# anneouyang/OuterSPACE

Hardware: AMD Instinct MI355X
Metric: spgemm_output_nnz_per_s (higher is better)
Workload: dtype f64

## Files before the change

outerspace_amd/csrc/osp_kernels.h:

```cpp
#pragma once
#include <type_traits>
#include "osp_prims.h"

namespace osp {

template <class T> struct TileCap;
#ifndef OSP_TILE_CAP_F32
#define OSP_TILE_CAP_F32 1792
#endif
template <> struct TileCap<float> { static constexpr int value = OSP_TILE_CAP_F32; };
#ifndef OSP_TILE_CAP_F64
#define OSP_TILE_CAP_F64 1536
#endif
template <> struct TileCap<double> { static constexpr int value = OSP_TILE_CAP_F64; };
constexpr int kMergeThreads = 256;
constexpr int kTileMaxRows = kMergeThreads - 1;
constexpr int kMulThreads = 256;
#ifndef OSP_MUL_PER_WAVE
#define OSP_MUL_PER_WAVE 2048
#endif
constexpr int kMulPerWave = OSP_MUL_PER_WAVE;
constexpr int kMulPerBlock = kMulPerWave * (kMulThreads / kWave);
#ifndef OSP_MUL_BATCH_MAX
#define OSP_MUL_BATCH_MAX 4096
// ... 1046 lines not shown
#ifdef OSP_MERGE_PROF
__device__ unsigned long long osp_merge_prof[16];
#define OSP_PROF_DECL __shared__ unsigned long long prof_acc[12]; if (tid < 12) prof_acc[tid] = 0; __syncthreads(); unsigned long long prof_t = clock64();
#define OSP_PROF_MARK(k) do { if (tid == 0) { const unsigned long long now_ = clock64(); prof_acc[k] += now_ - prof_t; prof_t = now_; } } while (0)
#define OSP_PROF_FLUSH do { if (tid == 0) for (int k_ = 0; k_ < 12; k_++) atomicAdd(&osp_merge_prof[k_], prof_acc[k_]); } while (0)
#else
#define OSP_PROF_DECL
#define OSP_PROF_MARK(k)
#define OSP_PROF_FLUSH
#endif

constexpr int kMergeMaxWgs = 5;
#ifndef OSP_TILE_ROUNDS
#define OSP_TILE_ROUNDS 3
#endif
constexpr int kTileRoundClasses = OSP_TILE_ROUNDS > 1 ? OSP_TILE_ROUNDS : 1;
static_assert(kTileRoundClasses <= 3, "OSP_TILE_ROUNDS: at most three bodies");
constexpr int tile_class_rounds(int lpt, int c, int K) { return (lpt * c + K - 1) / K; }
template <class T, int NT, int CAP, int MAXWG = kMergeMaxWgs, int ABL = 0>
constexpr int merge_wgs_per_cu() {
    const int wgs = (160 * 1024) / (int)(sizeof(MergeSmem<T, NT, CAP>) + ((ABL & 64) ? CAP * sizeof(T) : 0) + 64);
    return wgs > MAXWG ? MAXWG : wgs;
}
template <class T, int NT, int CAP, int MAXWG = kMergeMaxWgs, int ABL = 0>
constexpr int merge_waves_per_simd() {
    const int w = (merge_wgs_per_cu<T, NT, CAP, MAXWG, ABL>() * NT + 255) / 256;
    return w > 8 ? 8 : (w < 1 ? 1 : w);
}
template <class T, int NT, int ABL = 0, int CAP = TileCap<T>::value, int MAXWG = kMergeMaxWgs, bool RA = (OSP_RANK_ATOMIC != 0), bool GA = false>
__global__ __launch_bounds__(NT, (merge_waves_per_simd<T, NT, CAP, MAXWG, ABL>())) void merge_tiles_kernel(
    const TileDesc *__restrict__ desc, uint32_t ntiles, const MergeLevels<T> lvl, int colbits, uint64_t *tile_status,
    uint32_t *ticket, const uint64_t *__restrict__ out_base_p, uint32_t *__restrict__ c_col, T *__restrict__ c_val,
    uint64_t *__restrict__ out_end_p, const ChunkTable<T> ct = ChunkTable<T>{}, uint32_t nshards = 1, uint32_t *abort_word = nullptr,
    const GatherArgs<T> ga = GatherArgs<T>{}) {
    __shared__ MergeSmem<T, NT, CAP> sm;
    __shared__ TileDesc s_dnext;
    __shared__ uint32_t s_tnext;
    constexpr bool ROWWISE = (ABL & 64) != 0;
    __shared__ T rwval[ROWWISE ? CAP : 1];
    constexpr int kTileCap = CAP;
    constexpr int NW = NT / kWave;
    constexpr int LPT = (kTileCap + NT - 1) / NT;
    constexpr int ITERS = (kTileCap / NW + kWave - 1) / kWave;
    constexpr int DPT = (kDigits + NT - 1) / NT;
    static_assert(kTileMaxRows + 1 <= NT, "row offsets are fetched one per thread");
    unsigned tid = threadIdx.x, lane = lane_id(), w = tid >> 6;
    uint32_t shard = 0;
    if constexpr (GA) { if (tid < (uint32_t)kTileCap / 32u) sm.gbits[tid] = 0; }
    if (tid == 0) {
        if (nshards > 1) shard = atomicAdd(&ticket[nshards * kTicketStride], 1u) % nshards;
        const uint32_t t0 = (ABL & 4) ? blockIdx.x : take_ticket(ticket, nshards, shard, ntiles);
        s_tnext = t0;
        if (t0 < ntiles) s_dnext = desc[t0];
    }
    __syncthreads();
#ifndef OSP_TEST_NO_LATE_GUARD
    if (s_tnext >= ntiles) return;
#endif
    const uint64_t out_base = (ABL & 32) ? 0ull : *out_base_p;
    const uint32_t colmask = colbits < 32 ? ((1u << colbits) - 1u) : 0xffffffffu;
    uint32_t t = s_tnext;
    TileDesc d = s_dnext;
    OSP_CRUMB(5, ntiles, d.lvl, d.nr);
    uint64_t ro = 0;
    PartWords<T> lrec[LPT];
    static_assert(!GA || kTileCap % (NW * kWave) == 0, "gathered tiles: a wave's span is a whole number of wave-loads");
    static_assert(ITERS <= LPT, "sort passes: a wave's share of a full tile in LPT wave-loads");
// ... 51 lines not shown
        int64_t *__restrict__ c_rowptr = lvl.c_rowptr[d.lvl];
        const bool long_row = n > (uint32_t)kTileCap;
        uint32_t tn_reg = ntiles;
        if (long_row) {
            if (w == 0) {
                const uint64_t total = lvl.heavy_nnz[d.lvl][ra];
                const uint64_t excl = (ABL & 2) ? (uint64_t)t * kTileCap : lookback_prefix(tile_status, t, total, abort_word);
                if (lane == 0) {
                    tn_reg = (ABL & 4) ? t + gridDim.x : take_ticket(ticket, nshards, shard, ntiles);
                    c_rowptr[ra] = (int64_t)(out_base + excl);
                    if (t + 1 == ntiles) *out_end_p = out_base + excl + total;
                    s_tnext = tn_reg;
                    if (tn_reg < ntiles) s_dnext = desc[tn_reg];
                }
            }
            __syncthreads();
            t = s_tnext;
            d = s_dnext;
            request(d, t < ntiles);
            __syncthreads();
            continue;
        }
        auto tile_body = [&](auto rounds_tag) __attribute__((always_inline)) {
        constexpr int Q = decltype(rounds_tag)::value;
        static_assert(Q >= 1 && Q <= LPT, "rounds of a tile body");
        constexpr int SQ = K > 1 ? Q : ITERS;
        ix0 = GA ? w * (uint32_t)(kWave * Q) + lane : tid;
        int rowbits = 0;
        while ((1u << rowbits) < nr) rowbits++;
        const bool relkey = d.kbits != 0;
        const uint32_t cbase = d.cbase;
        const int keybits = relkey ? (int)d.kbits : colbits + rowbits;
        const int nbits = (n && !(ABL & 1)) ? keybits : 0;
        constexpr uint32_t HS = MergeSmem<T, NT, CAP>::kHashWords;
        typedef MergeSmem<T, NT, CAP> Smem;
        static_assert(!OSP_HASH_IN_CNT || offsetof(Smem, cnt) + sizeof(sm.cnt) == offsetof(Smem, pos0) + 4u * HS,
                      "hash table: from pos0 through the digit counters without a gap");
        uint32_t *htab = sm.htab();
        constexpr bool INPLACE = (ABL & 32) != 0;
        const bool early = nbits > 0 && keybits < 32 && !(ABL & 2) && !(ABL & 8) && !INPLACE;
        const bool gath = GA && d.rcnt != 0;
        uint32_t kq[LPT];
        T vq[LPT];
        uint32_t rq[(LPT + 1) / 2];
        constexpr bool kRunInPad = GA && Smem::kWide;
        constexpr bool kKeepPos = GA && Smem::kWide;
        uint32_t bpos[LPT];
        constexpr uint32_t GW = GA ? (uint32_t)kTileCap : 0u;
        constexpr uint32_t HSG = HS - GW;
        uint32_t *gsrc = htab, *htab_g = htab + GW;
        if constexpr (GA) {
            if (gath) {
                static_assert(HS > 2 * GW, "gathered tiles: the run table leaves a hash table of more than two words per entry... of half the entries");
                const uint32_t R = d.rcnt, tile0 = (uint32_t)(s + base);
                const RunDesc<T> *__restrict__ gruns = d.lvl ? ga.runs : ga.runs0;
                for (uint32_t x = tid; x < R; x += NT) {
                    uint32_t dst = lrec[0].w[0], src = lrec[0].w[1];
                    if (x == tid + NT) { dst = lrec[1].w[0]; src = lrec[1].w[1]; }
                    else if (x != tid) { const RunDesc<T> rd = gruns[d.rbeg + x]; dst = rd.dst; src = rd.src; }
                    const uint32_t st = dst - tile0;
                    gsrc[x] = src - st;
                    atomicOr(&sm.gbits[st >> 5], 1u << (st & 31u));
                }
                if (early) {
                    typedef uint32_t u32x4 __attribute__((ext_vector_type(4)));
                    static_assert((offsetof(Smem, pos0) + 4u * GW) % 16 == 0, "gathered tiles: the hash table starts 16-byte aligned");
// ... 33 lines not shown
                {
                    const uint32_t nwords = w * (2u * Q);
                    static_assert((NW - 1) * 2 * LPT <= kWave, "gathered tiles: the bits before a wave's span, one word per lane");
                    cnt0 = wave_reduce_sum<uint32_t>(lane < nwords ? (uint32_t)__popc(sm.gbits[lane]) : 0u);
                    cnt0 = (uint32_t)__builtin_amdgcn_readfirstlane((int)cnt0);
                }
#pragma unroll
                for (int q = 0; q < (LPT + 1) / 2; q++) rq[q] = 0;
#pragma unroll
                for (int q = 0; q < Q; q++) {
                    const uint32_t i = ix0 + q * ixs;
                    const uint32_t wi = w * (2u * Q) + 2u * (uint32_t)q;
                    const uint32_t mlo = sm.gbits[wi], mhi = sm.gbits[wi + 1];
                    const uint32_t below = __builtin_amdgcn_mbcnt_hi(mhi, __builtin_amdgcn_mbcnt_lo(mlo, 0u));
                    const uint32_t own = ((lane < 32 ? mlo >> lane : mhi >> (lane - 32)) & 1u);
                    const uint32_t r = cnt0 + below + own - 1u;
                    cnt0 += (uint32_t)__popc(mlo) + (uint32_t)__popc(mhi);
                    bpos[q] = i < n ? gsrc[r] + i : 0u;
                    rq[q >> 1] |= (i < n ? r : 0u) << (16 * (q & 1));
                }
                uint32_t bc[LPT];
#pragma unroll
                for (int q = 0; q < Q; q++) bc[q] = ga.b_colidx[bpos[q]];
#pragma unroll
                for (int q = 0; q < Q; q++) {
                    const uint32_t i = ix0 + q * ixs;
                    if (relkey) {
                        kq[q] = bc[q] - cbase;
                    } else {
                        uint32_t lo = 0, hi = nr;
                        while (hi - lo > 1) { const uint32_t mid = (lo + hi) >> 1; if (sm.rowo[mid] <= i) lo = mid; else hi = mid; }
                        kq[q] = (colbits < 32 ? (lo << colbits) : 0u) | bc[q];
                    }
                    if (i < n) sm.key0[i] = kq[q];
                }
                OSP_PROF_MARK(11);
                if (early) {
                    uint32_t hq[LPT], oq[LPT];
#pragma unroll
                    for (int q = 0; q < Q; q++) {
                        hq[q] = (uint32_t)(((uint64_t)(kq[q] * 2654435761u) * HSG) >> 32);
                        oq[q] = kq[q];
                        if (ix0 + q * ixs < n) oq[q] = atomicCAS(&htab_g[hq[q]], 0xffffffffu, kq[q]);
                    }
#pragma unroll
                    for (int q = 0; q < Q; q++) {
                        if (ix0 + q * ixs < n) {
                            uint32_t old = oq[q], h = hq[q];
                            while (old != 0xffffffffu && old != kq[q]) {
                                h = (h + 1 == HSG) ? 0u : h + 1;
                                old = atomicCAS(&htab_g[h], 0xffffffffu, kq[q]);
                            }
                            fresh += old == 0xffffffffu;
                        }
                    }
                }
            }
        }
        if (gath) {
        } else if (rw_tile) {
            if constexpr (ROWWISE) {
                constexpr uint32_t kRwGroup = 16, kRwSteps = 4, kRwUnroll = 4;
                const uint32_t c0 = ct.rowfirst[ra], c1 = ct.rowfirst[ra + nr];
                for (uint32_t cb = c0 + w * kRwGroup; cb < c1; cb += NW * kRwGroup) {
                    const uint32_t c = cb + lane;
                    const bool cv = lane < kRwGroup && c < c1;
                    const uint64_t o0 = cv ? ct.off[c] : 0ull, o1 = cv ? ct.off[c + 1] : 0ull;
// ... 5 lines not shown
                    {
                        uint32_t lo = 0, hi = nr;
                        while (hi - lo > 1) { const uint32_t mid = (lo + hi) >> 1; if (sm.rowo[mid] <= st) lo = mid; else hi = mid; }
                        lrow = colbits < 32 ? (lo << colbits) : 0u;
                    }
                    const uint32_t nvalid = min(kRwGroup, c1 - cb);
                    const uint32_t gbeg = wave_bcast(st, 0u), gend = wave_bcast(en, nvalid - 1);
                    for (uint32_t ib0 = gbeg; ib0 < gend; ib0 += kRwUnroll * kWave) {
                        uint32_t bcol[kRwUnroll], crow[kRwUnroll];
                        T bval[kRwUnroll], cav[kRwUnroll];
#pragma unroll
                        for (uint32_t u = 0; u < kRwUnroll; u++) {
                            const uint32_t i = ib0 + u * kWave + lane;
                            uint32_t lo = 0, hi = kRwGroup;
#pragma unroll
                            for (uint32_t step = 0; step < kRwSteps; step++) {
                                const uint32_t mid = (lo + hi) >> 1;
                                const uint32_t sv = (uint32_t)__shfl((int)st, (int)mid);
                                if (sv <= i) lo = mid; else hi = mid;
                            }
                            const uint32_t cst = (uint32_t)__shfl((int)st, (int)lo);
                            const uint32_t cbs = (uint32_t)__shfl((int)bsv, (int)lo);
                            crow[u] = (uint32_t)__shfl((int)lrow, (int)lo);
                            cav[u] = __shfl(av, (int)lo);
                            const uint32_t b = i < gend ? cbs + (i - cst) : 0u;
                            bcol[u] = ct.b_colidx[b];
                            bval[u] = ct.b_vals[b];
                        }
#pragma unroll
                        for (uint32_t u = 0; u < kRwUnroll; u++) {
                            const uint32_t i = ib0 + u * kWave + lane;
                            if (i < gend) {
                                const uint32_t key = crow[u] | bcol[u];
                                sm.key0[i] = key;
                                rwval[i] = cav[u] * bval[u];
                                if (early) {
                                    uint32_t h = (uint32_t)(((uint64_t)(key * 2654435761u) * HS) >> 32);
                                    uint32_t old = atomicCAS(&htab[h], 0xffffffffu, key);
                                    while (old != 0xffffffffu && old != key) {
                                        h = (h + 1 == HS) ? 0u : h + 1;
                                        old = atomicCAS(&htab[h], 0xffffffffu, key);
                                    }
                                    fresh += old == 0xffffffffu;
                                }
                            }
                        }
                    }
                }
            }
        } else {
#pragma unroll
            for (int q = 0; q < Q; q++) {
                const uint32_t i = ix0 + q * ixs;
                kq[q] = 0;
                if (i < n) {
                    if (relkey) {
                        kq[q] = lrec[q].col() - cbase;
                    } else {
                        uint32_t lo = 0, hi = nr;
                        while (hi - lo > 1) { const uint32_t mid = (lo + hi) >> 1; if (sm.rowo[mid] <= i) lo = mid; else hi = mid; }
                        kq[q] = (colbits < 32 ? (lo << colbits) : 0u) | lrec[q].col();
                    }
                    sm.key0[i] = kq[q];
                }
            }
            if (early) {
                uint32_t hq[LPT], oq[LPT];
#pragma unroll
                for (int q = 0; q < Q; q++) {
                    hq[q] = (uint32_t)(((uint64_t)(kq[q] * 2654435761u) * HS) >> 32);
                    oq[q] = kq[q];
                    if (ix0 + q * ixs < n) oq[q] = atomicCAS(&htab[hq[q]], 0xffffffffu, kq[q]);
                }
#pragma unroll
                for (int q = 0; q < Q; q++) {
                    if (ix0 + q * ixs < n) {
                        uint32_t old = oq[q], h = hq[q];
                        while (old != 0xffffffffu && old != kq[q]) {
                            h = (h + 1 == HS) ? 0u : h + 1;
                            old = atomicCAS(&htab[h], 0xffffffffu, kq[q]);
                        }
                        fresh += old == 0xffffffffu;
                    }
                }
            }
        }
        if (early) {
            const uint32_t wsum = wave_incl_scan(fresh);
            if (lane == kWave - 1 && wsum) atomicAdd(&sm.hcount, wsum);
        }
        const uint32_t per = K > 1 ? (uint32_t)(kWave * Q) : (n + NW - 1) / NW;
        const uint32_t wbeg = min(w * per, n), wend = min(wbeg + per, n);
        int cur = 0;
        __syncthreads();
        if constexpr (GA) {
            if (gath) {
                if (tid < (uint32_t)kTileCap / 32u) sm.gbits[tid] = 0;
                if constexpr (kRunInPad) {
#pragma unroll
                    for (int q = 0; q < Q; q++) {
                        const uint32_t i = ix0 + q * ixs;
                        if (i < n) sm.pad[i] = (uint16_t)(rq[q >> 1] >> (16 * (q & 1)));
                    }
                }
            }
        }
        OSP_PROF_MARK(1);
        if (early && tid == 0) lookback_publish(tile_status, t, sm.hcount);
        OSP_PROF_MARK(2);
        const int npass = (nbits + kDigitBits - 1) / kDigitBits;
        const int pbits = npass ? (nbits + npass - 1) / npass : 0;
        const uint32_t dmask = (1u << pbits) - 1u;
        const int ndig = 1 << pbits;
        for (int pass = 0, shift = 0; pass < npass; pass++, shift += pbits) {
            uint32_t *ksrc = sm.key(cur), *kdst = sm.key(cur ^ 1);
            uint16_t *psrc = sm.pos(cur), *pdst = sm.pos(cur ^ 1);
            if constexpr (ABL & 128) {
                for (int dd = lane; dd < ndig; dd += kWave) sm.cnt[w][dd] = 0;
            } else {
                uint64_t *c64 = reinterpret_cast<uint64_t *>(sm.cnt[w]);
                for (int dd = lane; dd < (ndig + 3) / 4; dd += kWave) c64[dd] = 0ull;
            }
            uint32_t kreg[SQ], rreg[SQ];
            auto rank_span = [&](auto bits_tag) {
                constexpr int BITS = decltype(bits_tag)::value;
#pragma unroll
                for (int it = 0; it < SQ; it++) {
                    const uint32_t i = wbeg + it * kWave + lane;
                    const bool valid = i < wend;
                    kreg[it] = valid ? ksrc[i] : 0u;
                    const unsigned dg = (kreg[it] >> shift) & dmask;
                    unsigned rk, cntd;
                    wave_match_digit<BITS>(dg, valid, rk, cntd);
                    rreg[it] = 0;
                    if (valid) {
                        const uint32_t c = sm.cnt[w][dg];
                        rreg[it] = c + rk;
                        if (rk == 0) sm.cnt[w][dg] = (uint16_t)(c + cntd);
                    }
                }
            };
            if constexpr (RA) {
            {
                uint32_t(*cnt32)[kDigits / 2] = reinterpret_cast<uint32_t(*)[kDigits / 2]>(sm.cnt);
#pragma unroll
                for (int it = 0; it < SQ; it++) {
                    const uint32_t i = wbeg + it * kWave + lane;
// ... 36 lines not shown
                const bool on = (int)tid * 4 < ndig;
                uint64_t pk[NW];
                uint32_t ssum = 0;
#pragma unroll
                for (int ww = 0; ww < NW; ww++) {
                    pk[ww] = on ? reinterpret_cast<const uint64_t *>(sm.cnt[ww])[tid] : 0ull;
                    ssum += (uint32_t)(pk[ww] & 0xffffu) + (uint32_t)((pk[ww] >> 16) & 0xffffu) + (uint32_t)((pk[ww] >> 32) & 0xffffu) +
                            (uint32_t)(pk[ww] >> 48);
                }
                uint32_t total;
                uint32_t ex = block_excl_scan<uint32_t, NT, false>(ssum, sm.scratch, &total)  ;
                if (on) {
                    uint32_t o[4][NW];
#pragma unroll
                    for (int q = 0; q < 4; q++) {
#pragma unroll
                        for (int ww = 0; ww < NW; ww++) { o[q][ww] = ex; ex += (uint32_t)(pk[ww] >> (16 * q)) & 0xffffu; }
                    }
#pragma unroll
                    for (int ww = 0; ww < NW; ww++)
                        reinterpret_cast<uint64_t *>(sm.cnt[ww])[tid] = (uint64_t)(o[0][ww] & 0xffffu) | ((uint64_t)(o[1][ww] & 0xffffu) << 16) |
                                                                        ((uint64_t)(o[2][ww] & 0xffffu) << 32) | ((uint64_t)(o[3][ww] & 0xffffu) << 48);
                }
            }
            __syncthreads();
            OSP_PROF_MARK(4);
#pragma unroll
            for (int it = 0; it < SQ; it++) {
                const uint32_t i = wbeg + it * kWave + lane;
                if (i < wend) {
                    const uint32_t k = kreg[it];
                    const uint32_t dst = (uint32_t)sm.cnt[w][(k >> shift) & dmask] + rreg[it];
                    kdst[dst] = k;
                    pdst[dst] = pass == 0 ? (uint16_t)i : psrc[i];
                }
            }
            cur ^= 1;
            __syncthreads();
            OSP_PROF_MARK(5);
        }
        uint32_t *skey = sm.key(cur);
        uint16_t *spos = sm.pos(cur);
        T *sval = rw_tile ? rwval : sm.vals(cur);
        if (npass == 0) {
            for (uint32_t i = tid; i < n; i += NT) spos[i] = (uint16_t)i;
        }
        OSP_CRUMB(2, npass, cur, nbits);
        if (!rw_tile && !gath) {
            const Part<T> *__restrict__ stg = lvl.stage[d.lvl];
#pragma unroll
            for (int q = 0; q < Q; q++) {
                const uint32_t i = ix0 + q * ixs;
                vq[q] = load_part_words(i < n ? &stg[s + i] : reinterpret_cast<const Part<T> *>(desc)).val();
            }
        }
        if constexpr (GA) {
            if (gath) {
                const uint32_t tile0 = (uint32_t)(s + base);
                const RunDesc<T> *__restrict__ gruns = d.lvl ? ga.runs : ga.runs0;
                T bv[LPT];
                if constexpr (kKeepPos) {
                    T av[LPT];
#pragma unroll
                    for (int q = 0; q < Q; q++) {
                        const uint32_t i = ix0 + q * ixs;
                        bv[q] = ga.b_vals[bpos[q]];
                        av[q] = gruns[d.rbeg + (i < n ? (uint32_t)sm.pad[i] : 0u)].av;
                    }
#pragma unroll
                    for (int q = 0; q < Q; q++) vq[q] = av[q] * bv[q];
                    (void)tile0;
                } else {
                RunDesc<T> rdq[LPT];
#pragma unroll
                for (int q = 0; q < Q; q++) {
                    const uint32_t i = ix0 + q * ixs;
                    uint32_t r;
                    if constexpr (kRunInPad) r = i < n ? (uint32_t)sm.pad[i] : 0u;
                    else r = (rq[q >> 1] >> (16 * (q & 1))) & 0xffffu;
                    rdq[q] = gruns[d.rbeg + r];
                }
#pragma unroll
                for (int q = 0; q < Q; q++) {
                    const uint32_t i = ix0 + q * ixs;
                    bv[q] = ga.b_vals[i < n ? rdq[q].src - (rdq[q].dst - tile0) + i : 0u];
                }
#pragma unroll
                for (int q = 0; q < Q; q++) vq[q] = rdq[q].av * bv[q];
                }
            }
        }
        if (npass == 0) __syncthreads();
        constexpr int IPT = Q;
        const uint32_t ib = tid * IPT;
        uint32_t heads = 0, hmask = 0;
#pragma unroll
        for (int q = 0; q < Q; q++) {
            const uint32_t i = ib + q;
            if (i < n) {
                const bool h = (i == 0) || (skey[i] != skey[i - 1]);
                hmask |= (h ? 1u : 0u) << q;
                heads += h;
            }
        }
        if constexpr (kRunInPad) {
            if (gath) __syncthreads();
        }
        if (!rw_tile) {
#pragma unroll
            for (int q = 0; q < Q; q++) {
                const uint32_t i = ix0 + q * ixs;
                if (i < n) sval[i] = vq[q];
            }
        }
        if (tid == 0) sm.nlongrun = 0;
        uint32_t total;
        uint32_t ex = block_excl_scan<uint32_t, NT, false>(heads, sm.scratch, &total);
        OSP_PROF_MARK(6);
        if (w == 0) {
            const uint64_t excl = INPLACE   ? 0ull
                                 : (ABL & 2) ? (uint64_t)t * kTileCap
                                 : early     ? lookback_prefix<false>(tile_status, t, total, abort_word)
                                             : lookback_prefix<true>(tile_status, t, total, abort_word);
            if (lane == 0) {
                sm.excl = excl;
                tn_reg = (ABL & 4) ? t + gridDim.x : take_ticket(ticket, nshards, shard, ntiles);
            }
        }
        OSP_PROF_MARK(7);
        const uint32_t oslot0 = ex;
#pragma unroll
        for (int q = 0; q < Q; q++) {
            const uint32_t i = ib + q;
            if (i < n) {
                sm.rank[i] = (uint16_t)ex;
                ex += (hmask >> q) & 1u;
            }
        }
        if (tid == 0) sm.rank[n] = (uint16_t)total;
        static_assert(IPT <= kRunShort, "the part of a run inside one thread's entries is never longer than a head's own share");
        T acc[IPT];
        uint32_t ocol[IPT], lmask = 0, tmask = 0;
        {
            T v[IPT];
#pragma unroll
            for (int q = 0; q < Q; q++) {
                const uint32_t i = ib + q;
                v[q] = i < n ? sval[spos[i]] : T(0);
            }
            T cur = T(0);
#pragma unroll
            for (int q = 0; q < Q; q++) {
                const uint32_t i = ib + q;
                const bool hd = (hmask >> q) & 1u;
                cur = hd ? v[q] : cur + v[q];
                const bool nexthd = q + 1 < IPT ? ((hmask >> (q + 1)) & 1u) != 0 : true;
                const bool tail = i < n && (i + 1 >= n || nexthd) && (hmask & ((2u << q) - 1u)) != 0;
                acc[q] = cur;
                ocol[q] = 0;
                tmask |= (tail ? 1u : 0u) << q;
            }
        }
        if (tmask) {
            const int qt = 31 - __builtin_clz(tmask);
            const uint32_t it = ib + (uint32_t)qt;
            if (qt == IPT - 1 && it + 1 < n) {
                const uint32_t ih = ib + (uint32_t)(31 - __builtin_clz(hmask));
                const uint32_t k = skey[it];
                T a = acc[IPT - 1];
                const uint32_t ulim = min(n, ih + (uint32_t)kRunShort);
                uint32_t u = it + 1;
                for (; u < ulim && skey[u] == k; u++) a += sval[spos[u]];
                if (u == ulim && u < n && skey[u] == k) {
                    const uint32_t idx = atomicAdd(&sm.nlongrun, 1u);
                    sm.long_sum()[idx] = a;
                    sm.long_pos()[idx] = (uint16_t)u;
                    lmask |= 1u << (IPT - 1);
                    a = index_as_value<T>(idx);
                }
                acc[IPT - 1] = a;
            }
#pragma unroll
            for (int q = 0; q < Q; q++) {
                if ((tmask >> q) & 1u) {
                    const uint32_t k = skey[ib + q];
                    ocol[q] = relkey ? k + cbase : (k & colmask);
                }
            }
        }
        if (tid == 0) s_tnext = tn_reg;
        __syncthreads();
        if (const uint32_t nlr = sm.nlongrun) {
            T *lsum = sm.long_sum();
            const uint16_t *lpos = sm.long_pos();
            for (uint32_t r = w; r < nlr; r += NW) {
                const uint32_t u1 = lpos[r], k = skey[u1];
                T a = lsum[r];
                for (uint32_t u0 = u1;; u0 += kWave) {
                    const uint32_t u = u0 + lane;
                    const bool in = u < n && skey[u] == k;
                    const T v = in ? sval[spos[u]] : T(0);
                    const uint64_t m = __ballot(in);
                    const uint32_t c = m == ~0ull ? (uint32_t)kWave : (uint32_t)__builtin_ctzll(~m);
                    for (uint32_t x = 0; x < c; x++) a += wave_bcast(v, x);
                    if (c < (uint32_t)kWave) break;
                }
                if (lane == 0) lsum[r] = a;
            }
            __syncthreads();
        }
        OSP_PROF_MARK(8);
#pragma unroll
        for (int q = 0; q < Q; q++) {
            if ((tmask >> q) & 1u) {
                const uint32_t slot = oslot0 + (uint32_t)__popc(hmask & ((2u << q) - 1u)) - 1u;
                skey[slot] = ocol[q];
                sval[slot] = ((lmask >> q) & 1u) ? sm.long_sum()[value_as_index<T>(acc[q])] : acc[q];
            }
        }
        if (tid == 0 && tn_reg < ntiles) s_dnext = desc[tn_reg];
        __syncthreads();
        OSP_PROF_MARK(9);
        const uint32_t tn = s_tnext;
        const TileDesc dn = s_dnext;
        OSP_CRUMB(3, total, tn, dn.s);
        request(dn, tn < ntiles);
        if constexpr (INPLACE) {
            Part<T> *outp = const_cast<Part<T> *>(lvl.stage[d.lvl]) + s;
            for (uint32_t o = tid; o < total; o += NT) outp[o] = Part<T>{skey[o], sval[o]};
            if (tid == 0) const_cast<uint32_t *>(lvl.heavy_nnz[d.lvl])[ra] = total;
        } else {
            const uint64_t obase = out_base + sm.excl;
            for (uint32_t o = tid; o < total; o += NT) {
                __builtin_nontemporal_store(skey[o], &c_col[obase + o]);
// ... 300 lines not shown
```

outerspace_amd/csrc/osp_pipeline.h:

```cpp
#pragma once

#define OSP_WITH_RA(ctx_, ...)                                               \
    do {                                                                     \
        if ((ctx_)->rank_atomic) { constexpr bool RA = true; __VA_ARGS__; }  \
        else { constexpr bool RA = false; __VA_ARGS__; }                     \
    } while (0)

template <class T> struct Producer {
    virtual ~Producer() {}
    virtual void produce(uint64_t r0, uint64_t r1, bool whole, uint64_t base, uint64_t count,
                         Part<T> *stage, PhaseTimer &tm, const uint32_t *cells = nullptr, Part<T> *qstage = nullptr,
                         const HubArgs *hub = nullptr, bool compact = false, bool has_long = true, bool desc_only = false, bool walk_all = false) = 0;
};

template <class T> struct MergeIO {
    Part<T> *stage;
    const uint64_t *row_off; uint64_t r0, r1, base;
    int64_t *c_rowptr; uint32_t *c_col; T *c_val;
    const uint64_t *out_in; uint64_t *out_out;
    ChunkTable<T> ct{};
    uint32_t *abort_word = nullptr;
    const RunDesc<T> *runs0 = nullptr; const uint32_t *rowfirst0 = nullptr; const uint32_t *b_colidx = nullptr; const T *b_vals = nullptr;
};
template <class T> struct ShortRuns {
// ... 322 lines not shown
            pl.hub.sx = ds->hub.sx;
            res->info.hub_plan_launches++;
            res->info.hub_cells += ncells;
            res->info.hub_rows += pl.mode_rows[kModeStretch];
            res->info.hub_partials += pl.mode_partials[kModeStretch];
        }
        dbg_sync(s, "plan of the hub rows");
    }
    if (ds && ds->expand_rows) {
        pl.expand_ok = true;
        const bool hubs = pl.hub.cells != nullptr;
        const uint64_t rows_x = pl.mode_rows[kModeSplitRow] + (hubs ? 0 : pl.mode_rows[kModeStretch]);
        pl.xpartials = pl.mode_partials[kModeSplitRow] + (hubs ? 0 : pl.mode_partials[kModeStretch]);
        if (rows_x) {
            pl.xjobbase = sc.get<uint64_t>((uint64_t)nlong + 1);
            device_exclusive_scan<ExpandJobs, uint64_t>(ExpandJobs{pl.p0.long_rows, row_off, pl.hmode, kModeSplitRow, hubs ? kModeSplitRow : kModeStretch},
                                                        nlong, pl.xjobbase, pl.hscan_tmp, s);
            pl.xjobs_bound = pl.xpartials / kExpandJob + rows_x;
        }
    }
}

template <class T>
static void merge_panel(Context *ctx, Result *res, PhaseTimer &tm, const MergeIO<T> &io, int colbits, PanelPlan<T> &pl) {
    hipStream_t s = ctx->stream;
    Scratch &sc = pl.sc;
    constexpr uint32_t kCap = (uint32_t)TileCap<T>::value;
    const uint32_t max_rows = pl.max_rows;
#ifdef OSP_CHECK_DESC
    crumbs_init();
#endif
    const uint64_t r1 = io.r1, base = io.base;
    const TilePlan &p0 = pl.p0;

    MergeLevels<T> lv{};
    lv.stage[0] = io.stage; lv.row_off[0] = io.row_off; lv.base[0] = base; lv.c_rowptr[0] = io.c_rowptr; lv.heavy_nnz[0] = nullptr;
    uint32_t ntot = p0.ntiles;
    TileDesc *desc = nullptr;
    TilePlan p1;
    uint64_t *vbase = pl.vbase;
    int64_t *vptr = nullptr;
    uint64_t *seg_src = nullptr;
    uint32_t *seg_nnz = nullptr;
    Part<T> *qstage = pl.qstage;
    if (p0.nlong) {
        const uint32_t nlong = p0.nlong;
        uint64_t *hoff = pl.hoff, *hscan_tmp = pl.hscan_tmp, *blkbase = pl.blkbase, *hbase = pl.hbase;
        uint8_t *hbits = pl.hbits;
        uint32_t *nstretch = pl.nstretch, *ghist = pl.ghist, *ghist_tmp = pl.ghist_tmp;
        const uint64_t nh = pl.nh, nblocks = pl.nblocks, nvirt = pl.nvirt, ncell = pl.ncell;
        uint64_t *vrow_off = pl.vrow_off;
        uint8_t *vfirst = pl.vfirst;
        if (pl.mode_rows[kModeSplitRow]) {
            tm.begin(PH_SPLIT_K);
            OSP_WITH_RA(ctx, split_row_kernel<T, RA><<<nlong, kSplitRowThreads, 0, s>>>(p0.long_rows, nlong, hbits, pl.hmode, vbase, hoff, io.row_off,
                                                                                     base, colbits, io.stage, qstage, vrow_off));
            tm.end(PH_SPLIT_K);
            res->info.split_launches++;
            res->info.split_partials += pl.mode_partials[kModeSplitRow];
            dbg_sync(s, "split: one-workgroup rows");
        }
        if (nblocks && !pl.hub.cells) {
            split_count_kernel<<<(unsigned)nblocks, kSplitThreads, 0, s>>>(p0.long_rows, nlong, blkbase, hbase, hbits, nstretch, io.row_off,
                                                                         base, colbits, (const char *)io.stage, (uint32_t)sizeof(Part<T>), ghist);
            device_exclusive_scan<LoadU32, uint32_t>(LoadU32{ghist}, ncell, ghist, ghist_tmp, s);
            OSP_WITH_RA(ctx, split_scatter_kernel<T, RA><<<(unsigned)nblocks, kSplitThreads, 0, s>>>(
// ... 36 lines not shown
                        dense_segment_kernel<T, true><<<grid_for(ndense, kDenseWaves), kDenseWaves * kWave, 0, s>>>(dense_list, ndense, vrow_off, pl.vcol0, pl.vcol1,
                                                                              qstage, seg_nnz);
                    else
                        dense_segment_kernel<T, false><<<grid_for(ndense, kDenseWaves), kDenseWaves * kWave, 0, s>>>(dense_list, ndense, vrow_off, pl.vcol0, pl.vcol1,
                                                                              qstage, seg_nnz);
                    res->info.dense_segments += ndense;
                    rest_list = others;
                    nrest = nseg_long - ndense;
                }
            }
            dbg_sync(s, "over-long segments: dense accumulation");
            const uint32_t big_cap = getenv("OSP_BIGTILE_CAP") ? std::min<uint32_t>((uint32_t)strtoul(getenv("OSP_BIGTILE_CAP"), nullptr, 10), kBigTileCap)
                                                                : (uint32_t)kBigTileCap;
            uint32_t nhuge = 0, nmid = 0;
            uint32_t *huge_list = nullptr, *mid_list = nullptr;
            if (nrest) {
                const SegHugeFlag hf{rest_list, vrow_off, big_cap};
                device_exclusive_scan<SegHugeFlag, uint32_t>(hf, nrest, hscan, (uint32_t *)sscan_tmp, s);
                nhuge = d2h(hscan + nrest, s);
                nmid = nrest - nhuge;
                huge_list = sc.get<uint32_t>(nhuge);
                mid_list = sc.get<uint32_t>(nmid);
                seg_partition_kernel<<<grid_for(nrest, 256), 256, 0, s>>>(hf, hscan, nrest, huge_list, mid_list);
            }
            res->info.sorted_segments += nhuge;
            if (nmid) {
                TileDesc *bdesc = sc.get<TileDesc>(nmid);
                seg_tile_desc_kernel<<<grid_for(nmid, 256), 256, 0, s>>>(mid_list, nmid, vrow_off, pl.vcol0, pl.vcol1, bdesc);
                uint32_t *bticket = sc.get<uint32_t>(1);
                zero_async(s, {{bticket, sizeof(uint32_t)}});
                const uint32_t bgrid = ctx->cus * (uint32_t)merge_wgs_per_cu<T, kBigTileThreads, kBigTileCap>();
                OSP_WITH_RA(ctx, merge_tiles_kernel<T, kBigTileThreads, 32, kBigTileCap, kMergeMaxWgs, RA>
                            <<<std::min<uint32_t>(nmid, bgrid), kBigTileThreads, 0, s>>>(bdesc, nmid, lv, colbits, nullptr, bticket, nullptr, nullptr,
                                                                                         nullptr, nullptr));
            }
            dbg_sync(s, "over-long segments: big in-place tiles");
            if (nhuge) {
                uint64_t *soff = sc.get<uint64_t>((uint64_t)nhuge + 1);
                device_exclusive_scan<HeavyLen, uint64_t>(HeavyLen{huge_list, vrow_off}, nhuge, soff, sscan_tmp, s);
                const uint64_t ns = d2h(soff + nhuge, s);
                res->info.sorted_partials += ns;
                uint64_t *keys[2] = {sc.get<uint64_t>(ns + 1), sc.get<uint64_t>(ns + 1)};
                uint32_t *poss[2] = {sc.get<uint32_t>(ns), sc.get<uint32_t>(ns)};
                uint32_t *hist = sc.get<uint32_t>(sort_hist_entries(ns));
                uint32_t *hist_tmp = sc.get<uint32_t>(scan_scratch_entries(sort_hist_entries(ns)));
                heavy_fill_kernel<<<grid_for(ns, 256), 256, 0, s>>>(huge_list, soff, nhuge, vrow_off, 0, colbits, (const char *)qstage,
                                                                    (uint32_t)sizeof(Part<T>), ns, keys[0], poss[0]);
                const int cur = device_radix_sort_pairs<uint64_t>(keys, poss, ns, colbits + bits_for(nhuge), hist, hist_tmp, s, ctx->rank_atomic);
                T *sorted_val = sc.get<T>(ns);
                heavy_gather_kernel<T><<<grid_for(ns, 256), 256, 0, s>>>(poss[cur], qstage, ns, sorted_val);
                uint64_t *headscan = sc.get<uint64_t>(ns + 1);
                uint64_t *headscan_tmp = sc.get<uint64_t>(scan_scratch_entries(ns));
                device_exclusive_scan<HeavyHeadFlag, uint64_t>(HeavyHeadFlag{keys[cur]}, ns, headscan, headscan_tmp, s);
                uint64_t *head_pos = keys[cur ^ 1];
                heavy_heads_kernel<<<grid_for(ns + 1, 256), 256, 0, s>>>(keys[cur], headscan, ns, head_pos);
                heavy_reduce_kernel<T><<<grid_for(ns, 256), 256, 0, s>>>(keys[cur], sorted_val, headscan, head_pos, ns, huge_list, soff,
                                                                         nhuge, vrow_off, 0, colbits, qstage);
                heavy_rows_kernel<<<grid_for(nhuge, 256), 256, 0, s>>>(huge_list, soff, nhuge, headscan, seg_nnz);
            }
            dbg_sync(s, "over-long segments: global sort");
            heavy_src_inplace_kernel<<<grid_for(nseg_long, 256), 256, 0, s>>>(p1.long_rows, nseg_long, vrow_off, 0, seg_src);
        }
        lv.heavy_nnz[1] = seg_nnz;
        uint32_t *j0 = sc.get<uint32_t>(nlong), *tb = sc.get<uint32_t>((uint64_t)nlong + 1), *extra = sc.get<uint32_t>((uint64_t)nlong + 1);
        chain_rows_kernel<<<grid_for(nlong + 1, 256), 256, 0, s>>>(p0.long_rows, nlong, p0.tile_rows, p0.ntiles, vbase, p1.tile_rows,
                                                                  p1.ntiles, j0, tb, extra);
        device_exclusive_scan<LoadU32, uint32_t>(LoadU32{extra}, nlong, extra, (uint32_t *)hscan_tmp, s);
        ntot = p0.ntiles + (p1.ntiles - nlong);
        desc = sc.get<TileDesc>(ntot);
        tile_desc_kernel<(int)kCap><<<grid_for(p0.ntiles, 256), 256, 0, s>>>(p0.tile_rows, p0.ntiles, r1, io.row_off, base, 0u, j0, extra,
                                                                           nlong, tb, pl.vcol0, pl.vcol1, desc, nullptr, nullptr, io.rowfirst0);
        tile_desc_kernel<(int)kCap><<<grid_for(p1.ntiles, 256), 256, 0, s>>>(p1.tile_rows, p1.ntiles, nvirt, vrow_off, 0, 1u, j0, extra,
                                                                           nlong, tb, pl.vcol0, pl.vcol1, desc, pl.ga.runs ? pl.vrun_off : nullptr,
                                                                           pl.vrun_end);
        dbg_sync(s, "tile chain");
    } else {
        desc = sc.get<TileDesc>(ntot);
        tile_desc_kernel<(int)kCap><<<grid_for(p0.ntiles, 256), 256, 0, s>>>(p0.tile_rows, p0.ntiles, r1, io.row_off, base, 0u, nullptr,
                                                                           nullptr, 0u, nullptr, nullptr, nullptr, desc, nullptr, nullptr, io.rowfirst0);
    }
    uint64_t *tile_status = sc.get<uint64_t>(ntot);
    const uint32_t nshards = 1u;
    uint32_t *ticket = sc.get<uint32_t>((uint64_t)(nshards + 1) * kTicketStride);
    zero_async(s, {{tile_status, (uint64_t)ntot * sizeof(uint64_t)}, {ticket, (uint64_t)(nshards + 1) * kTicketStride * sizeof(uint32_t)}});
    dbg_sync(s, "tile planning, splits, over-long segments");
    tm.begin(PH_MERGE_K);
    if (io.ct.enabled) {
        const uint32_t rw_grid = ctx->cus * (uint32_t)merge_wgs_per_cu<T, kMergeThreads, TileCap<T>::value, kMergeMaxWgs, 64>();
        OSP_WITH_RA(ctx, merge_tiles_kernel<T, kMergeThreads, 64, TileCap<T>::value, kMergeMaxWgs, RA>
                    <<<std::min<uint32_t>(ntot, rw_grid), kMergeThreads, 0, s>>>(desc, ntot, lv, colbits, tile_status, ticket, io.out_in, io.c_col,
                                                                                 io.c_val, io.out_out, io.ct, nshards, io.abort_word));
    } else if (pl.ga.runs || io.runs0) {
        GatherArgs<T> ga = pl.ga;
        ga.runs0 = io.runs0;
        if (io.runs0) { ga.b_colidx = io.b_colidx; ga.b_vals = io.b_vals; }
        const uint32_t merge_grid = ctx->cus * (uint32_t)merge_wgs_per_cu<T, kMergeThreads, TileCap<T>::value>();
        OSP_WITH_RA(ctx, merge_tiles_kernel<T, kMergeThreads, 0, TileCap<T>::value, kMergeMaxWgs, RA, true>
                    <<<std::min<uint32_t>(ntot, merge_grid), kMergeThreads, 0, s>>>(desc, ntot, lv, colbits, tile_status, ticket, io.out_in, io.c_col,
                                                                                    io.c_val, io.out_out, ChunkTable<T>{}, nshards, io.abort_word, ga));
    } else {
        const uint32_t merge_grid = ctx->cus * (uint32_t)merge_wgs_per_cu<T, kMergeThreads, TileCap<T>::value>();
        OSP_WITH_RA(ctx, merge_tiles_kernel<T, kMergeThreads, 0, TileCap<T>::value, kMergeMaxWgs, RA>
                    <<<std::min<uint32_t>(ntot, merge_grid), kMergeThreads, 0, s>>>(desc, ntot, lv, colbits, tile_status, ticket, io.out_in, io.c_col,
                                                                                    io.c_val, io.out_out, ChunkTable<T>{}, nshards, io.abort_word));
    }
    tm.end(PH_MERGE_K);
    dbg_sync(s, "merge tiles");
#ifdef OSP_MERGE_PROF
    if (getenv("OSP_VERBOSE")) {
        std::vector<TileDesc> hd(ntot);
        copy_d2h(hd.data(), desc, (size_t)ntot * sizeof(TileDesc), s);
        uint64_t byp[5] = {0}, ent[5] = {0}, gt = 0, ge = 0, gr = 0, bits[33] = {0};
        for (const TileDesc &t : hd) {
            if (t.n > kCap) continue;
            int rb = 0; while ((1u << rb) < t.nr) rb++;
            const int kb = t.kbits ? (int)t.kbits : colbits + rb;
            const int np = std::min(4, (kb + kDigitBits - 1) / kDigitBits);
            byp[np]++; ent[np] += t.n; bits[std::min(kb, 32)] += 1;
            if (t.rcnt) { gt++; ge += t.n; gr += t.rcnt; }
        }
        fprintf(stderr, "[osp]   tiles by sort passes:");
        for (int k = 0; k < 5; k++) if (byp[k]) fprintf(stderr, " %d passes: %llu tiles, %.0f entries each;", k, (unsigned long long)byp[k], (double)ent[k] / byp[k]);
        fprintf(stderr, " gathered: %llu tiles, %.0f entries and %.1f runs each\n[osp]   tiles by key bits:", (unsigned long long)gt, gt ? (double)ge / gt : 0.0, gt ? (double)gr / gt : 0.0);
        for (int k = 0; k <= 32; k++) if (bits[k]) fprintf(stderr, " %d: %llu;", k, (unsigned long long)bits[k]);
        constexpr int lpt = ((int)kCap + kMergeThreads - 1) / kMergeThreads;
        uint64_t byq[lpt + 1] = {0}, slots = 0, need = 0, run = 0;
        for (const TileDesc &t : hd) {
            if (t.n > kCap) continue;
            const int q = std::max(1, (int)((t.n + kMergeThreads - 1) / kMergeThreads));
            int body = lpt;
            for (int c = kTileRoundClasses; c >= 1; c--) if (q <= tile_class_rounds(lpt, c, kTileRoundClasses)) body = tile_class_rounds(lpt, c, kTileRoundClasses);
            byq[q]++; slots += lpt; need += q; run += body;
        }
        fprintf(stderr, "\n[osp]   tiles by rounds (Q = ceil(n / %d)):", kMergeThreads);
        for (int q = 1; q <= lpt; q++) fprintf(stderr, " Q=%d: %llu;", q, (unsigned long long)byq[q]);
        fprintf(stderr, " slot-rounds needed %.1f %%, run %.1f %% of %d per tile (%d bodies)", slots ? 100.0 * need / slots : 0.0,
                slots ? 100.0 * run / slots : 0.0, lpt, kTileRoundClasses);
        fprintf(stderr, "\n");
    }
    if (getenv("OSP_VERBOSE")) {
        unsigned long long hp[16] = {0}, z[16] = {0};
        OSP_HIP(hipStreamSynchronize(s));
        (void)hipMemcpyFromSymbol(hp, HIP_SYMBOL(osp_merge_prof), sizeof(hp));
        (void)hipMemcpyToSymbol(HIP_SYMBOL(osp_merge_prof), z, sizeof(z));
        static const char *names[12] = {"run table / hash init", "keys + hash count", "publish", "rank", "digit scan", "scatter", "values + heads + scan",
                                        "look-back + ticket", "run sums", "compaction", "output + next tile's request", "gathered: lookup + columns"};
        double tot = 0;
        for (int k = 0; k < 12; k++) tot += (double)hp[k];
        fprintf(stderr, "[osp]   merge kernel, %u tiles, cycles of thread 0 per phase:", ntot);
        for (int k = 0; k < 12; k++) fprintf(stderr, " %s %.1f %%;", names[k], 100.0 * hp[k] / tot);
        fprintf(stderr, " %.0f cycles per tile and workgroup\n", tot / std::max(1u, ntot));
    }
#endif
    res->info.merge_launches++;
    if (p1.nlong) {
        heavy_copy_kernel<T><<<grid_for(p1.nlong, 8), 256, 0, s>>>(p1.long_rows, p1.nlong, seg_src, seg_nnz, vptr, qstage, nullptr, nullptr,
                                                                   io.c_col, io.c_val);
// ... 357 lines not shown
```

Before: 68.41 billion.

## Pack tile positions into low bits of sort keys in merge tiles

After: 69.02 billion (median of 6 runs). About the same (+0.9%).

```diff
diff --git a/outerspace_amd/csrc/osp_kernels.h b/outerspace_amd/csrc/osp_kernels.h
--- a/outerspace_amd/csrc/osp_kernels.h
+++ b/outerspace_amd/csrc/osp_kernels.h
@@ -1102,7 +1102,7 @@
     const TileDesc *__restrict__ desc, uint32_t ntiles, const MergeLevels<T> lvl, int colbits, uint64_t *tile_status,
     uint32_t *ticket, const uint64_t *__restrict__ out_base_p, uint32_t *__restrict__ c_col, T *__restrict__ c_val,
     uint64_t *__restrict__ out_end_p, const ChunkTable<T> ct = ChunkTable<T>{}, uint32_t nshards = 1, uint32_t *abort_word = nullptr,
-    const GatherArgs<T> ga = GatherArgs<T>{}) {
+    const GatherArgs<T> ga = GatherArgs<T>{}, uint32_t tile_packed = 1) {
     __shared__ MergeSmem<T, NT, CAP> sm;
     __shared__ TileDesc s_dnext;
     __shared__ uint32_t s_tnext;
@@ -1220,6 +1220,11 @@
         const uint32_t cbase = d.cbase;
         const int keybits = relkey ? (int)d.kbits : colbits + rowbits;
         const int nbits = (n && !(ABL & 1)) ? keybits : 0;
+        constexpr int PB = 32 - __builtin_clz((unsigned)(kTileCap - 1));
+        static_assert((1u << PB) >= (unsigned)kTileCap && PB < 16, "packed tiles: a position fits PB bits");
+        const bool pk = __builtin_amdgcn_readfirstlane((int)(tile_packed != 0 && keybits + PB <= 32)) != 0;
+        const int pb = pk ? PB : 0;
+        const uint32_t pmask = (1u << pb) - 1u;
         constexpr uint32_t HS = MergeSmem<T, NT, CAP>::kHashWords;
         typedef MergeSmem<T, NT, CAP> Smem;
         static_assert(!OSP_HASH_IN_CNT || offsetof(Smem, cnt) + sizeof(sm.cnt) == offsetof(Smem, pos0) + 4u * HS,
@@ -1319,7 +1324,7 @@
                         while (hi - lo > 1) { const uint32_t mid = (lo + hi) >> 1; if (sm.rowo[mid] <= i) lo = mid; else hi = mid; }
                         kq[q] = (colbits < 32 ? (lo << colbits) : 0u) | bc[q];
                     }
-                    if (i < n) sm.key0[i] = kq[q];
+                    if (i < n) sm.key0[i] = (kq[q] << pb) | (i & pmask);
                 }
                 OSP_PROF_MARK(11);
                 if (early) {
@@ -1391,7 +1396,7 @@
                             const uint32_t i = ib0 + u * kWave + lane;
                             if (i < gend) {
                                 const uint32_t key = crow[u] | bcol[u];
-                                sm.key0[i] = key;
+                                sm.key0[i] = (key << pb) | (i & pmask);
                                 rwval[i] = cav[u] * bval[u];
                                 if (early) {
                                     uint32_t h = (uint32_t)(((uint64_t)(key * 2654435761u) * HS) >> 32);
@@ -1420,7 +1425,7 @@
                         while (hi - lo > 1) { const uint32_t mid = (lo + hi) >> 1; if (sm.rowo[mid] <= i) lo = mid; else hi = mid; }
                         kq[q] = (colbits < 32 ? (lo << colbits) : 0u) | lrec[q].col();
                     }
-                    sm.key0[i] = kq[q];
+                    sm.key0[i] = (kq[q] << pb) | (i & pmask);
                 }
             }
             if (early) {
@@ -1471,7 +1476,8 @@
         const int pbits = npass ? (nbits + npass - 1) / npass : 0;
         const uint32_t dmask = (1u << pbits) - 1u;
         const int ndig = 1 << pbits;
-        for (int pass = 0, shift = 0; pass < npass; pass++, shift += pbits) {
+        for (int pass = 0, kshift = 0; pass < npass; pass++, kshift += pbits) {
+            const int shift = kshift + pb;
             uint32_t *ksrc = sm.key(cur), *kdst = sm.key(cur ^ 1);
             uint16_t *psrc = sm.pos(cur), *pdst = sm.pos(cur ^ 1);
             if constexpr (ABL & 128) {
@@ -1574,7 +1580,7 @@
                     const uint32_t k = kreg[it];
                     const uint32_t dst = (uint32_t)sm.cnt[w][(k >> shift) & dmask] + rreg[it];
                     kdst[dst] = k;
-                    pdst[dst] = pass == 0 ? (uint16_t)i : psrc[i];
+                    if (!pk) pdst[dst] = pass == 0 ? (uint16_t)i : psrc[i];
                 }
             }
             cur ^= 1;
@@ -1584,7 +1590,7 @@
         uint32_t *skey = sm.key(cur);
         uint16_t *spos = sm.pos(cur);
         T *sval = rw_tile ? rwval : sm.vals(cur);
-        if (npass == 0) {
+        if (npass == 0 && !pk) {
             for (uint32_t i = tid; i < n; i += NT) spos[i] = (uint16_t)i;
         }
         OSP_CRUMB(2, npass, cur, nbits);
@@ -1636,11 +1642,15 @@
         constexpr int IPT = Q;
         const uint32_t ib = tid * IPT;
         uint32_t heads = 0, hmask = 0;
+        uint32_t sw[IPT];
 #pragma unroll
         for (int q = 0; q < Q; q++) {
             const uint32_t i = ib + q;
+            sw[q] = 0;
             if (i < n) {
-                const bool h = (i == 0) || (skey[i] != skey[i - 1]);
+                sw[q] = skey[i];
+                const uint32_t prev = q ? sw[q - 1] : skey[i ? i - 1 : 0];
+                const bool h = (i == 0) || ((sw[q] ^ prev) >> pb) != 0;
                 hmask |= (h ? 1u : 0u) << q;
                 heads += h;
             }
@@ -1685,10 +1695,15 @@
         uint32_t ocol[IPT], lmask = 0, tmask = 0;
         {
             T v[IPT];
-#pragma unroll
-            for (int q = 0; q < Q; q++) {
-                const uint32_t i = ib + q;
-                v[q] = i < n ? sval[spos[i]] : T(0);
+            if (pk) {
+#pragma unroll
+                for (int q = 0; q < Q; q++) v[q] = ib + q < n ? sval[sw[q] & pmask] : T(0);
+            } else {
+#pragma unroll
+                for (int q = 0; q < Q; q++) {
+                    const uint32_t i = ib + q;
+                    v[q] = i < n ? sval[spos[i]] : T(0);
+                }
             }
             T cur = T(0);
 #pragma unroll
@@ -1708,12 +1723,12 @@
             const uint32_t it = ib + (uint32_t)qt;
             if (qt == IPT - 1 && it + 1 < n) {
                 const uint32_t ih = ib + (uint32_t)(31 - __builtin_clz(hmask));
-                const uint32_t k = skey[it];
+                const uint32_t k = sw[IPT - 1] >> pb;
                 T a = acc[IPT - 1];
                 const uint32_t ulim = min(n, ih + (uint32_t)kRunShort);
-                uint32_t u = it + 1;
-                for (; u < ulim && skey[u] == k; u++) a += sval[spos[u]];
-                if (u == ulim && u < n && skey[u] == k) {
+                uint32_t u = it + 1, wu = 0;
+                for (; u < ulim && ((wu = skey[u]) >> pb) == k; u++) a += sval[pk ? (wu & pmask) : (uint32_t)spos[u]];
+                if (u == ulim && u < n && (skey[u] >> pb) == k) {
                     const uint32_t idx = atomicAdd(&sm.nlongrun, 1u);
                     sm.long_sum()[idx] = a;
                     sm.long_pos()[idx] = (uint16_t)u;
@@ -1725,7 +1740,7 @@
 #pragma unroll
             for (int q = 0; q < Q; q++) {
                 if ((tmask >> q) & 1u) {
-                    const uint32_t k = skey[ib + q];
+                    const uint32_t k = sw[q] >> pb;
                     ocol[q] = relkey ? k + cbase : (k & colmask);
                 }
             }
@@ -1736,12 +1751,13 @@
             T *lsum = sm.long_sum();
             const uint16_t *lpos = sm.long_pos();
             for (uint32_t r = w; r < nlr; r += NW) {
-                const uint32_t u1 = lpos[r], k = skey[u1];
+                const uint32_t u1 = lpos[r], k = skey[u1] >> pb;
                 T a = lsum[r];
                 for (uint32_t u0 = u1;; u0 += kWave) {
                     const uint32_t u = u0 + lane;
-                    const bool in = u < n && skey[u] == k;
-                    const T v = in ? sval[spos[u]] : T(0);
+                    const uint32_t wu = u < n ? skey[u] : 0u;
+                    const bool in = u < n && (wu >> pb) == k;
+                    const T v = in ? sval[pk ? (wu & pmask) : (uint32_t)spos[u]] : T(0);
                     const uint64_t m = __ballot(in);
                     const uint32_t c = m == ~0ull ? (uint32_t)kWave : (uint32_t)__builtin_ctzll(~m);
                     for (uint32_t x = 0; x < c; x++) a += wave_bcast(v, x);
diff --git a/outerspace_amd/csrc/osp_pipeline.h b/outerspace_amd/csrc/osp_pipeline.h
--- a/outerspace_amd/csrc/osp_pipeline.h
+++ b/outerspace_amd/csrc/osp_pipeline.h
@@ -378,6 +378,7 @@
 #endif
     const uint64_t r1 = io.r1, base = io.base;
     const TilePlan &p0 = pl.p0;
+    const uint32_t tile_packed = !(getenv("OSP_TILE_PACKED") && atoi(getenv("OSP_TILE_PACKED")) == 0);
 
     MergeLevels<T> lv{};
     lv.stage[0] = io.stage; lv.row_off[0] = io.row_off; lv.base[0] = base; lv.c_rowptr[0] = io.c_rowptr; lv.heavy_nnz[0] = nullptr;
@@ -480,7 +481,8 @@
                 const uint32_t bgrid = ctx->cus * (uint32_t)merge_wgs_per_cu<T, kBigTileThreads, kBigTileCap>();
                 OSP_WITH_RA(ctx, merge_tiles_kernel<T, kBigTileThreads, 32, kBigTileCap, kMergeMaxWgs, RA>
                             <<<std::min<uint32_t>(nmid, bgrid), kBigTileThreads, 0, s>>>(bdesc, nmid, lv, colbits, nullptr, bticket, nullptr, nullptr,
-                                                                                         nullptr, nullptr));
+                                                                                         nullptr, nullptr, ChunkTable<T>{}, 1u, nullptr,
+                                                                                         GatherArgs<T>{}, tile_packed));
             }
             dbg_sync(s, "over-long segments: big in-place tiles");
             if (nhuge) {
@@ -537,7 +539,8 @@
         const uint32_t rw_grid = ctx->cus * (uint32_t)merge_wgs_per_cu<T, kMergeThreads, TileCap<T>::value, kMergeMaxWgs, 64>();
         OSP_WITH_RA(ctx, merge_tiles_kernel<T, kMergeThreads, 64, TileCap<T>::value, kMergeMaxWgs, RA>
                     <<<std::min<uint32_t>(ntot, rw_grid), kMergeThreads, 0, s>>>(desc, ntot, lv, colbits, tile_status, ticket, io.out_in, io.c_col,
-                                                                                 io.c_val, io.out_out, io.ct, nshards, io.abort_word));
+                                                                                 io.c_val, io.out_out, io.ct, nshards, io.abort_word, GatherArgs<T>{},
+                                                                                 tile_packed));
     } else if (pl.ga.runs || io.runs0) {
         GatherArgs<T> ga = pl.ga;
         ga.runs0 = io.runs0;
@@ -545,12 +548,14 @@
         const uint32_t merge_grid = ctx->cus * (uint32_t)merge_wgs_per_cu<T, kMergeThreads, TileCap<T>::value>();
         OSP_WITH_RA(ctx, merge_tiles_kernel<T, kMergeThreads, 0, TileCap<T>::value, kMergeMaxWgs, RA, true>
                     <<<std::min<uint32_t>(ntot, merge_grid), kMergeThreads, 0, s>>>(desc, ntot, lv, colbits, tile_status, ticket, io.out_in, io.c_col,
-                                                                                    io.c_val, io.out_out, ChunkTable<T>{}, nshards, io.abort_word, ga));
+                                                                                    io.c_val, io.out_out, ChunkTable<T>{}, nshards, io.abort_word, ga,
+                                                                                    tile_packed));
     } else {
         const uint32_t merge_grid = ctx->cus * (uint32_t)merge_wgs_per_cu<T, kMergeThreads, TileCap<T>::value>();
         OSP_WITH_RA(ctx, merge_tiles_kernel<T, kMergeThreads, 0, TileCap<T>::value, kMergeMaxWgs, RA>
                     <<<std::min<uint32_t>(ntot, merge_grid), kMergeThreads, 0, s>>>(desc, ntot, lv, colbits, tile_status, ticket, io.out_in, io.c_col,
-                                                                                    io.c_val, io.out_out, ChunkTable<T>{}, nshards, io.abort_word));
+                                                                                    io.c_val, io.out_out, ChunkTable<T>{}, nshards, io.abort_word,
+                                                                                    GatherArgs<T>{}, tile_packed));
     }
     tm.end(PH_MERGE_K);
     dbg_sync(s, "merge tiles");
@@ -558,7 +563,8 @@
     if (getenv("OSP_VERBOSE")) {
         std::vector<TileDesc> hd(ntot);
         copy_d2h(hd.data(), desc, (size_t)ntot * sizeof(TileDesc), s);
-        uint64_t byp[5] = {0}, ent[5] = {0}, gt = 0, ge = 0, gr = 0, bits[33] = {0};
+        uint64_t byp[5] = {0}, ent[5] = {0}, gt = 0, ge = 0, gr = 0, bits[33] = {0}, npk = 0, epk = 0, nall = 0, eall = 0;
+        constexpr int pos_bits = 32 - __builtin_clz(kCap - 1u);
         for (const TileDesc &t : hd) {
             if (t.n > kCap) continue;
             int rb = 0; while ((1u << rb) < t.nr) rb++;
@@ -566,11 +572,15 @@
             const int np = std::min(4, (kb + kDigitBits - 1) / kDigitBits);
             byp[np]++; ent[np] += t.n; bits[std::min(kb, 32)] += 1;
             if (t.rcnt) { gt++; ge += t.n; gr += t.rcnt; }
+            nall++; eall += t.n;
+            if (tile_packed && kb + pos_bits <= 32) { npk++; epk += t.n; }
         }
         fprintf(stderr, "[osp]   tiles by sort passes:");
         for (int k = 0; k < 5; k++) if (byp[k]) fprintf(stderr, " %d passes: %llu tiles, %.0f entries each;", k, (unsigned long long)byp[k], (double)ent[k] / byp[k]);
         fprintf(stderr, " gathered: %llu tiles, %.0f entries and %.1f runs each\n[osp]   tiles by key bits:", (unsigned long long)gt, gt ? (double)ge / gt : 0.0, gt ? (double)gr / gt : 0.0);
         for (int k = 0; k <= 32; k++) if (bits[k]) fprintf(stderr, " %d: %llu;", k, (unsigned long long)bits[k]);
+        fprintf(stderr, "\n[osp]   packed tiles (key bits + %d <= 32): %llu of %llu (%.1f %%), %.1f %% of their entries", pos_bits, (unsigned long long)npk,
+                (unsigned long long)nall, nall ? 100.0 * npk / nall : 0.0, eall ? 100.0 * epk / eall : 0.0);
         constexpr int lpt = ((int)kCap + kMergeThreads - 1) / kMergeThreads;
         uint64_t byq[lpt + 1] = {0}, slots = 0, need = 0, run = 0;
         for (const TileDesc &t : hd) {
```
